# givemeone1astkiss/RNA-MPNN

Measured on AMD Instinct MI355X. Metric: nucleotides/sec (forward), k=30 RNA graphs, higher is better.
Workload: dtype bf16; 1 GPU; C2: batch=256 RNAs, n~U[100,140], k=30, default 10-layer RNAMPNN, P=T; max_len=140, weights=closed-form deterministic init (3,536,900 params), parallelism=dp1

## Files before the change

rna-mpnn_amd/csrc/kernels_mpnn.hip:

```cpp
#include "kernels_bf16.h"
#include "bf16_dev.h"
#include <cstdlib>

static_assert(RN_E_F16 == 1 && RN_P_F16 == 1, "k_resmpnn works on f16 e and f16 P / Q tables");
#if !defined(RN_EXPERIMENTS) && (defined(RM_EXP_NOQ) || defined(RM_EXP_NOESTORE) || defined(RM_EXP_NOELOAD) || defined(RM_EXP_NOMFMA) || defined(RM_EXP_NOGELU) || \
                                 defined(RM_EXP_NOLDS) || defined(RM_EXP_STAGGER) || defined(RM_EXP_PRIO) || defined(RM_WAVES) || defined(RM_RING8) || defined(RM_EDB) || \
                                 defined(RM_QROLL) || defined(RM_NO_EPI_FENCE) || defined(RM_EXP_FWDSWEEP))
#error "experimental variants of k_resmpnn need -DRN_EXPERIMENTS (tools/build_mpnn_variant.sh)"
#endif

#ifndef RM_WAVES
#define RM_WAVES 8
#endif
#if RM_WAVES <= 8 && !defined(RM_QROLL)
#define RM_QFULL 1
#endif
#define RM_LDS_P 131072
#define RM_LDS_BE (RM_LDS_P + RM_WAVES * 1024)
#define RM_LDS_BM (RM_LDS_BE + 512)
#define RM_LDS_GB (RM_LDS_BM + 512)
#define RM_LDS_Z (RM_LDS_GB + 512 + 128)
#define RM_LDS_CTR (RM_LDS_Z + 512)
#define RM_LDS_B0 (RM_LDS_CTR + 16)
#define RM_LDS_BYTES (RM_LDS_B0 + 512)
static_assert(RM_LDS_Z % 256 == 128 && RM_LDS_BYTES <= 160 * 1024, "LDS layout");

__device__ __forceinline__ u32x4* rm_efrag(bf16_t* e, int blk, int lane) { return reinterpret_cast<u32x4*>(e) + (size_t)blk * 512 + lane; }
__device__ __forceinline__ f32x16 rm_ld16(const unsigned char* smem, unsigned off) {
    const f32x4* p = reinterpret_cast<const f32x4*>(smem + off);
    const f32x4 a = p[0], b = p[1], c = p[2], d = p[3];
    return f32x16{a[0], a[1], a[2], a[3], b[0], b[1], b[2], b[3], c[0], c[1], c[2], c[3], d[0], d[1], d[2], d[3]};
}
__device__ __forceinline__ float rm_fma_ll(f16x2 a, f16x2 b, float c) {
    float d;
    asm("v_fma_mix_f32 %0, %1, %2, %3 op_sel_hi:[1,1,0]" : "=v"(d) : "v"(a), "v"(b), "v"(c));
    return d;
}
__device__ __forceinline__ float rm_fma_hh(f16x2 a, f16x2 b, float c) {
    float d;
    asm("v_fma_mix_f32 %0, %1, %2, %3 op_sel:[1,1,0] op_sel_hi:[1,1,0]" : "=v"(d) : "v"(a), "v"(b), "v"(c));
    return d;
}
__device__ __forceinline__ f16x4 rm_h4(unsigned w0, unsigned w1) {
    typedef __attribute__((ext_vector_type(2))) unsigned u32x2_;
    return __builtin_bit_cast(f16x4, u32x2_{w0, w1});
}

#ifdef RM_EXP_NOGELU
#define phi4s(y) (y)
#endif
template <bool DO_EDGE, bool DO_MSG, bool EMBED = false>
__global__ void __launch_bounds__(RM_WAVES * 64, RM_WAVES / 4) k_resmpnn(PackInfo pk, int k, int reverse, const int* __restrict__ nbr, bf16_t* __restrict__ e,
        const bf16_t* __restrict__ p_e, const bf16_t* __restrict__ q_e, const bf16_t* __restrict__ p_m, const bf16_t* __restrict__ q_m,
        const float* __restrict__ h_res, const bf16_t* __restrict__ img_e_g, const float* __restrict__ b2e,
        const bf16_t* __restrict__ img_m_g, const float* __restrict__ b2m, float* __restrict__ agg,
        const float* __restrict__ geomh = nullptr, const float* __restrict__ ee_b0 = nullptr) {
    static_assert(!EMBED || (!DO_EDGE && DO_MSG), "EMBED: the edge embedding (feature.py:386-571) in front of the message of layer 1");
    extern __shared__ __attribute__((aligned(256))) unsigned char smem[];
    u32x4* img_e = reinterpret_cast<u32x4*>(smem);
    u32x4* img_m = img_e + 4096;
    constexpr int NW = RM_WAVES;
    const int tid = threadIdx.x, wave = tid >> 6, lane = tid & 63, r = lane & 31, h = lane >> 5;
    const int ntot = pk.cu[pk.B];
    const int nblocks = ntot;
    const int zero_row = pk.Nmax;
    const bool slot_ok = r < k;
    const int last_idx = ntot * k - 1;

    int blk_end, stride, first, lo = 0;
    if ((gridDim.x & 7) == 0) {
        const int chunk = (nblocks + 7) >> 3, x = blockIdx.x & 7;
        blk_end = min(nblocks, (x + 1) * chunk);
        stride = (gridDim.x >> 3) * NW;
        lo = x * chunk;
        first = lo + (blockIdx.x >> 3) * NW;
    } else {
        blk_end = nblocks; stride = gridDim.x * NW; first = blockIdx.x * NW;
    }
    const int mirror = lo + blk_end - 1;
    auto phys = [&](int b) -> int { return __builtin_amdgcn_readfirstlane(reverse ? mirror - b : b); };
    int* lds_ctr = reinterpret_cast<int*>(smem + RM_LDS_CTR);
    auto claim_issue = [&]() -> int {
        int v = 0;
        if (lane == 0) v = __hip_atomic_fetch_add(lds_ctr, 1, __ATOMIC_RELAXED, __HIP_MEMORY_SCOPE_WORKGROUP);
        return v;
    };
    auto claim_block = [&](int v) -> int {
        const int n = __builtin_amdgcn_readfirstlane(v);
        return first + (n % NW) + (n / NW) * stride;
    };
    int blk = first + wave, nxt = blk + stride;
    u32x4 ef[8];
    unsigned pn_e = 0u, pn_m = 0u;
    int jraw = -1;
    const int b0 = __builtin_amdgcn_readfirstlane(blk < blk_end ? (reverse ? mirror - blk : blk) : 0);
    if (nblocks > 0) {
        const int i0 = b0 * k + r;
        jraw = nbr[i0 > last_idx ? last_idx : i0];
        if (!EMBED) {
#pragma unroll
            for (int s = 0; s < 8; ++s) ef[s] = rm_efrag(e, b0, lane)[64 * s];
        }
        if (DO_EDGE) pn_e = reinterpret_cast<const unsigned*>(p_e + (size_t)b0 * RN_D)[lane];
        if (DO_MSG) pn_m = reinterpret_cast<const unsigned*>(p_m + (size_t)b0 * RN_D)[lane];
    }
    if (DO_EDGE) stage_image_dma<NW * 64>(img_e, reinterpret_cast<const u32x4*>(img_e_g), tid);
    if (EMBED) stage_image_dma<NW * 64, (4 * EMB_KS + 32) * 64>(img_e, reinterpret_cast<const u32x4*>(img_e_g), tid);
    if (DO_MSG) stage_image_dma<NW * 64>(img_m, reinterpret_cast<const u32x4*>(img_m_g), tid);
    if (EMBED && tid >= 256 + 64 && tid < 256 + 64 + 128) reinterpret_cast<float*>(smem + RM_LDS_B0)[tid - 320] = kGA * ee_b0[tid - 320];
    if (tid < 128) {
        reinterpret_cast<float*>(smem + RM_LDS_BE)[tid] = (DO_EDGE || EMBED) ? b2e[tid] : 0.f;
        const float bm = DO_MSG ? b2m[tid] : 0.f;
        const f16x2 bh = cvt_h2(bm, bm);
        reinterpret_cast<unsigned*>(smem + RM_LDS_BM)[tid] = __builtin_bit_cast(unsigned, bh);
        const f16x2 ph = phi2s(bh);
        reinterpret_cast<float*>(smem + RM_LDS_GB)[tid] = (float)bh[0] * (float)ph[0];
    } else if (tid < 256) {
        reinterpret_cast<unsigned*>(smem + RM_LDS_Z)[tid - 128] = 0u;
    } else if (tid == 256) {
        *lds_ctr = 2 * NW;
    }
    dma_landed();
    __syncthreads();
    if (blk >= blk_end) return;

    const unsigned off_pe = RM_LDS_P + wave * 1024 + 64 * h, off_pm = off_pe + 512, off_be = RM_LDS_BE + 64 * h;
    float* lds_pw = reinterpret_cast<float*>(smem + RM_LDS_P + wave * 1024);
    auto stage_p = [&]() {
        if (DO_EDGE) {
            const f16x2 v = __builtin_bit_cast(f16x2, pn_e);
            *reinterpret_cast<f32x2*>(lds_pw + 2 * lane) = f32x2{(float)v[0], (float)v[1]};
        }
        if (DO_MSG) {
            const f16x2 v = __builtin_bit_cast(f16x2, pn_m);
            *reinterpret_cast<f32x2*>(lds_pw + 128 + 2 * lane) = f32x2{(float)v[0], (float)v[1]};
        }
    };
    constexpr int C_FIRST = DO_EDGE ? 0 : 8, C_LAST = DO_MSG ? 15 : 7;
#ifdef RM_EXP_NOLDS
#define RM_FRAG(c, s) (wf[s])
#else
#define RM_FRAG(c, s) (((c) < 8 ? img_e : img_m)[(((c) >> 2) & 1) * 2048 + (((c) & 3) * 8 + (s)) * 64 + lane])
#endif
#define RM_NEXT(c) ((c) == C_LAST ? C_FIRST : (c) + 1)
#define RM_FENCE() __builtin_amdgcn_sched_barrier(0)
#ifdef RM_NO_EPI_FENCE
#define RM_EFENCE() do { } while (0)
#else
#define RM_EFENCE() RM_FENCE()
#endif
#ifdef RM_RING8
#define RM_RING 8
#else
#define RM_RING 4
#endif
    u32x4 q[8], hb[8], wf[8];
    f32x16 T;
    auto gather_q = [&](auto cbc, const bf16_t* table, int jj) {
        constexpr int cb = decltype(cbc)::value;
        const int row = jj >= 0 ? (jj > zero_row ? zero_row : jj) : zero_row;
        const u32x4* src = reinterpret_cast<const u32x4*>(table + (size_t)row * RN_D + 32 * cb + 16 * h);
#ifdef RM_EXP_NOQ
        (void)src; q[2 * cb] = u32x4{0u, 0u, 0u, 0u}; q[2 * cb + 1] = u32x4{0u, 0u, 0u, 0u};
#else
        q[2 * cb] = src[0]; q[2 * cb + 1] = src[1];
#endif
    };
    auto chain = [&](auto cc, auto&& extra) {
        constexpr int c = decltype(cc)::value, kind = c >> 2, cn = RM_NEXT(c);
#pragma unroll
        for (int s = RM_RING; s < 8; ++s) wf[s] = RM_FRAG(c, s);
        RM_FENCE();
        static_for<8>([&](auto sc) {
            constexpr int s = decltype(sc)::value;
#ifdef RM_EXP_NOMFMA
            if constexpr (s == 0) T[0] += __uint_as_float(wf[s][0] ^ (kind == 0 || kind == 2 ? ef[s][0] : hb[s][0]));
            else T[s] += __uint_as_float(wf[s][0] ^ (kind == 0 || kind == 2 ? ef[s][0] : hb[s][0]));
#else
            if constexpr (kind == 3) {
                if constexpr (s == 0) T = mfma32h(hb[0], wf[0], f32x16{0.f, 0.f, 0.f, 0.f, 0.f, 0.f, 0.f, 0.f, 0.f, 0.f, 0.f, 0.f, 0.f, 0.f, 0.f, 0.f});
                else T = mfma32h(hb[s], wf[s], T);
            } else if constexpr (kind == 1) T = mfma32h(wf[s], hb[s], T);
            else T = mfma32h(wf[s], ef[s], T);
#endif
            if constexpr (s < RM_RING) wf[s] = RM_FRAG(cn, s);
            extra(sc);
        });
        asm volatile("" : "+v"(T) :: "memory");
    };
    auto no_extra = [](auto) {};
#ifdef RM_QFULL
#define RM_GQ_ROLL(cb, tab, jj) do { } while (0)
#define RM_GQ_FULL(tab, jj) do { gather_q(std::integral_constant<int, 0>{}, tab, jj); gather_q(std::integral_constant<int, 1>{}, tab, jj); gather_q(std::integral_constant<int, 2>{}, tab, jj); gather_q(std::integral_constant<int, 3>{}, tab, jj); } while (0)
#else
#define RM_GQ_ROLL(cb, tab, jj) gather_q(cb, tab, jj)
#define RM_GQ_FULL(tab, jj) do { } while (0)
#endif
    auto cvt_tile = [&](f16x4 (&x)[4], int next_init) {
#pragma unroll
        for (int v = 0; v < 4; ++v) x[v] = cvt_h4(T[4 * v], T[4 * v + 1], T[4 * v + 2], T[4 * v + 3]);
        asm volatile("" : "+v"(x[0]), "+v"(x[1]), "+v"(x[2]), "+v"(x[3]) :: "memory");
#ifndef RM_EXP_NOLDS
        if (next_init >= 0) T = rm_ld16(smem, (unsigned)next_init);
#endif
    };
    auto epi_first = [&](auto cbc, int next_init) {
        constexpr int cb = decltype(cbc)::value;
        f16x4 x[4];
        cvt_tile(x, next_init);
#pragma unroll
        for (int v = 0; v < 4; ++v) {
            const f16x4 y = x[v] + rm_h4(q[2 * cb + (v >> 1)][2 * (v & 1)], q[2 * cb + (v >> 1)][2 * (v & 1) + 1]);
            const f16x4 g = y * phi4s(y);
            hb[2 * cb + (v >> 1)][2 * (v & 1)] = __builtin_bit_cast(unsigned, lo2(g));
            hb[2 * cb + (v >> 1)][2 * (v & 1) + 1] = __builtin_bit_cast(unsigned, hi2(g));
        }
        RM_EFENCE();
    };
    auto epi_edge = [&](auto obc, int next_init, int gblk) {
        constexpr int ob = decltype(obc)::value;
        f16x4 x[4];
        cvt_tile(x, next_init);
#pragma unroll
        for (int v = 0; v < 4; ++v) {
            const f16x4 ph = phi4s(x[v]);
            const int sp = v >> 1, t = 2 * (v & 1);
            const unsigned o0 = ef[2 * ob + sp][t], o1 = ef[2 * ob + sp][t + 1];
            ef[2 * ob + sp][t] = __builtin_bit_cast(unsigned, __builtin_elementwise_fma(lo2(x[v]), lo2(ph), __builtin_bit_cast(f16x2, o0)));
            ef[2 * ob + sp][t + 1] = __builtin_bit_cast(unsigned, __builtin_elementwise_fma(hi2(x[v]), hi2(ph), __builtin_bit_cast(f16x2, o1)));
#ifndef RM_EXP_NOESTORE
            if (v & 1) rm_efrag(e, gblk, lane)[64 * (2 * ob + sp)] = ef[2 * ob + sp];
#endif
        }
        RM_EFENCE();
    };
    auto epi_mean = [&](auto nbc, int next_init, int gblk, float cabs, float inv, float hres) {
        constexpr int nb = decltype(nbc)::value;
        const unsigned bw = reinterpret_cast<const unsigned*>(smem + RM_LDS_BM)[32 * nb + r];
        const float gbv = reinterpret_cast<const float*>(smem + RM_LDS_GB)[32 * nb + r];
        f16x4 x[4];
        cvt_tile(x, next_init);
        const f16x4 bh = rm_h4(bw, bw);
        float s0 = 0.f, s1 = 0.f;
#pragma unroll
        for (int v = 0; v < 4; ++v) {
            const f16x4 y = x[v] + bh;
            const f16x4 ph = phi4s(y);
            s0 = rm_fma_ll(lo2(y), lo2(ph), s0);
            s1 = rm_fma_hh(lo2(y), lo2(ph), s1);
            s0 = rm_fma_ll(hi2(y), hi2(ph), s0);
            s1 = rm_fma_hh(hi2(y), hi2(ph), s1);
        }
        float sum = s0 + s1;
        sum += __shfl_xor(sum, 32, 64);
        agg[(size_t)gblk * RN_D + 32 * nb + r] = fmaf(sum - cabs * gbv, inv, hres);
        RM_EFENCE();
    };

    f32x4 nrec[7];
    auto load_rec = [&](int jj) {
        const f32x4* src = reinterpret_cast<const f32x4*>(geomh + (size_t)(jj >= 0 ? jj : 0) * RN_GEOMH + 32 * h);
#pragma unroll
        for (int v = 0; v < 7; ++v) nrec[v] = src[v];
    };
    int j = (slot_ok && b0 < ntot) ? jraw : -1;
    if constexpr (EMBED) load_rec(j);
    gather_q(std::integral_constant<int, 0>{}, DO_EDGE ? q_e : q_m, j);
    gather_q(std::integral_constant<int, 1>{}, DO_EDGE ? q_e : q_m, j);
#ifdef RM_QFULL
    gather_q(std::integral_constant<int, 2>{}, DO_EDGE ? q_e : q_m, j);
    gather_q(std::integral_constant<int, 3>{}, DO_EDGE ? q_e : q_m, j);
#endif
    stage_p();
#pragma unroll
    for (int s = 0; s < RM_RING; ++s) wf[s] = RM_FRAG(C_FIRST, s);
    if constexpr (!EMBED) T = rm_ld16(smem, j >= 0 ? (DO_EDGE ? off_pe : off_pm) : (unsigned)RM_LDS_Z);
    RM_FENCE();

#ifdef RM_EXP_STAGGER
    if (wave >= NW / 2) { for (int i = 0; i < RM_EXP_STAGGER; ++i) __builtin_amdgcn_s_sleep(4); }
#endif
#ifdef RM_EXP_PRIO
    if (wave >= NW / 2) __builtin_amdgcn_s_setprio(RM_EXP_PRIO);
#endif
    while (true) {
        const int nblk = nxt;
        const int claim_v = claim_issue();
        const bool has_next = nblk < blk_end;
        const int pblk = phys(blk);
        const int nb_c = phys(has_next ? nblk : blk);
        const int in_ = nb_c * k + r;
        const int jn_raw = nbr[in_ > last_idx ? last_idx : in_];
        if (DO_EDGE) pn_e = reinterpret_cast<const unsigned*>(p_e + (size_t)nb_c * RN_D)[lane];
        if (DO_MSG) pn_m = reinterpret_cast<const unsigned*>(p_m + (size_t)nb_c * RN_D)[lane];
        const bool valid = j >= 0;
        const unsigned vmask = (unsigned)(__ballot(valid) & 0xffffffffull);
        const int cnt = __popc(vmask);
        const float cabs = (float)(32 - cnt);
        const float inv = cnt > 0 ? kGAi * __builtin_amdgcn_rcpf((float)cnt) : 0.f;
        const int a_pe = valid ? (int)off_pe : RM_LDS_Z, a_pm = valid ? (int)off_pm : RM_LDS_Z, a_be = valid ? (int)off_be : RM_LDS_Z;
        const int jn = (slot_ok && nb_c < ntot) ? jn_raw : -1;
        const int a_next = jn >= 0 ? (int)(DO_EDGE ? off_pe : off_pm) : RM_LDS_Z;
#ifdef RM_EDB
        u32x4 efn[8];
#pragma unroll
        for (int s = 0; s < 8; ++s) efn[s] = rm_efrag(e, nb_c, lane)[64 * s];
#endif
        using I0 = std::integral_constant<int, 0>; using I1 = std::integral_constant<int, 1>;
        using I2 = std::integral_constant<int, 2>; using I3 = std::integral_constant<int, 3>;
        RM_FENCE();

        if constexpr (DO_EDGE) {
            chain(std::integral_constant<int, 0>{}, no_extra); RM_GQ_ROLL(I2{}, q_e, j); epi_first(I0{}, a_pe + 128);
            chain(std::integral_constant<int, 1>{}, no_extra); RM_GQ_ROLL(I3{}, q_e, j); epi_first(I1{}, a_pe + 256);
            chain(std::integral_constant<int, 2>{}, no_extra); epi_first(I2{}, a_pe + 384);
            chain(std::integral_constant<int, 3>{}, no_extra); epi_first(I3{}, a_be);
            chain(std::integral_constant<int, 4>{}, no_extra); if constexpr (DO_MSG) RM_GQ_FULL(q_m, j); epi_edge(I0{}, a_be + 128, pblk);
            chain(std::integral_constant<int, 5>{}, no_extra); epi_edge(I1{}, a_be + 256, pblk);
            if constexpr (DO_MSG) {
                chain(std::integral_constant<int, 6>{}, no_extra); RM_GQ_ROLL(I0{}, q_m, j); epi_edge(I2{}, a_be + 384, pblk);
                chain(std::integral_constant<int, 7>{}, no_extra); RM_GQ_ROLL(I1{}, q_m, j); epi_edge(I3{}, a_pm, pblk);
            } else {
                chain(std::integral_constant<int, 6>{}, no_extra); epi_edge(I2{}, a_be + 384, pblk);
                chain(std::integral_constant<int, 7>{}, no_extra);
                stage_p();
                epi_edge(I3{}, a_next, pblk);
                RM_GQ_ROLL(I0{}, q_e, jn); RM_GQ_ROLL(I1{}, q_e, jn); RM_GQ_FULL(q_e, jn);
#pragma unroll
                for (int s = 0; s < 8; ++s) ef[s] = rm_efrag(e, nb_c, lane)[64 * s];
            }
        }
        if constexpr (EMBED) {
            const float* __restrict__ gc = geomh + (size_t)pblk * RN_GEOMH;
            auto catom = [&](int a, int d) { return a < 4 ? gc[3 * a + d] : gc[32 + 3 * (a - 4) + d]; };
            auto cbond = [&](int a, int d) { return a < 3 ? gc[12 + 3 * a + d] : gc[32 + 12 + 3 * (a - 3) + d]; };
            auto cnorm = [&](int a, int d) { return a < 2 ? gc[21 + 3 * a + d] : gc[32 + 21 + 3 * (a - 2) + d]; };
            float nl[28];
#pragma unroll
            for (int v = 0; v < 7; ++v) { nl[4 * v] = nrec[v][0]; nl[4 * v + 1] = nrec[v][1]; nl[4 * v + 2] = nrec[v][2]; nl[4 * v + 3] = nrec[v][3]; }
            float ft[EMB_SLOTS];
#pragma unroll
            for (int a = 0; a < 7; ++a) {
                const float ax = catom(a, 0), ay = catom(a, 1), az = catom(a, 2);
#pragma unroll
                for (int bl = 0; bl < 4; ++bl) {
                    const float dx = nl[3 * bl] - ax, dy = nl[3 * bl + 1] - ay, dz = nl[3 * bl + 2] - az;
                    ft[4 * a + bl] = __builtin_amdgcn_sqrtf(fmaf(dz, dz, fmaf(dy, dy, fmaf(dx, dx, kSEPS))));
                }
            }
#pragma unroll
            for (int a = 0; a < 5; ++a) {
                const float ax = cbond(a, 0), ay = cbond(a, 1), az = cbond(a, 2);
#pragma unroll
                for (int bl = 0; bl < 3; ++bl) ft[28 + 3 * a + bl] = fmaf(az, nl[12 + 3 * bl + 2], fmaf(ay, nl[12 + 3 * bl + 1], ax * nl[12 + 3 * bl]));
            }
#pragma unroll
            for (int a = 0; a < 4; ++a) {
                const float ax = cnorm(a, 0), ay = cnorm(a, 1), az = cnorm(a, 2);
#pragma unroll
                for (int bl = 0; bl < 2; ++bl) ft[43 + 2 * a + bl] = fmaf(az, nl[21 + 3 * bl + 2], fmaf(ay, nl[21 + 3 * bl + 1], ax * nl[21 + 3 * bl]));
            }
#pragma unroll
            for (int pz = 51; pz < EMB_SLOTS; ++pz) ft[pz] = 0.f;
            u32x4 xf[EMB_KS];
#pragma unroll
            for (int s7 = 0; s7 < EMB_KS; ++s7)
#pragma unroll
                for (int t = 0; t < 4; ++t) xf[s7][t] = p_pack2(ft[8 * s7 + 2 * t], ft[8 * s7 + 2 * t + 1]);
            RM_FENCE();
            const unsigned emask = valid ? 0xffffffffu : 0u;
            static_for<4>([&](auto mbc) {
                constexpr int mb = decltype(mbc)::value;
                T = rm_ld16(smem, RM_LDS_B0 + 128 * mb + 64 * h);
#pragma unroll
                for (int s7 = 0; s7 < EMB_KS; ++s7) T = mfma32h(img_e[(mb * EMB_KS + s7) * 64 + lane], xf[s7], T);
                asm volatile("" : "+v"(T) :: "memory");
#pragma unroll
                for (int v = 0; v < 4; ++v) {
                    const f16x4 x = cvt_h4(T[4 * v], T[4 * v + 1], T[4 * v + 2], T[4 * v + 3]);
                    const f16x4 g = x * phi4s(x);
                    hb[2 * mb + (v >> 1)][2 * (v & 1)] = __builtin_bit_cast(unsigned, lo2(g));
                    hb[2 * mb + (v >> 1)][2 * (v & 1) + 1] = __builtin_bit_cast(unsigned, hi2(g));
                }
                RM_FENCE();
            });
            static_for<4>([&](auto obc) {
                constexpr int ob = decltype(obc)::value;
                T = rm_ld16(smem, RM_LDS_BE + 128 * ob + 64 * h);
#pragma unroll
                for (int ks = 0; ks < 8; ++ks) T = mfma32h(img_e[(4 * EMB_KS + ob * 8 + ks) * 64 + lane], hb[ks], T);
                asm volatile("" : "+v"(T) :: "memory");
#pragma unroll
                for (int v = 0; v < 4; ++v) {
                    const f16x4 x = cvt_h4(T[4 * v], T[4 * v + 1], T[4 * v + 2], T[4 * v + 3]);
                    const f16x4 g = x * phi4s(x);
                    const int sp = v >> 1, t = 2 * (v & 1);
                    ef[2 * ob + sp][t] = __builtin_bit_cast(unsigned, lo2(g)) & emask;
                    ef[2 * ob + sp][t + 1] = __builtin_bit_cast(unsigned, hi2(g)) & emask;
                    if (v & 1) rm_efrag(e, pblk, lane)[64 * (2 * ob + sp)] = ef[2 * ob + sp];
                }
                RM_FENCE();
            });
            T = rm_ld16(smem, (unsigned)a_pm);
            RM_FENCE();
        }
        if constexpr (DO_MSG) {
            chain(std::integral_constant<int, 8>{}, no_extra); RM_GQ_ROLL(I2{}, q_m, j); epi_first(I0{}, a_pm + 128);
            chain(std::integral_constant<int, 9>{}, no_extra); RM_GQ_ROLL(I3{}, q_m, j); epi_first(I1{}, a_pm + 256);
            chain(std::integral_constant<int, 10>{}, no_extra); epi_first(I2{}, a_pm + 384);
            chain(std::integral_constant<int, 11>{}, [&](auto sc) {
#if !defined(RM_EXP_NOELOAD) && !defined(RM_EDB)
                if constexpr (!EMBED) { constexpr int s = decltype(sc)::value; ef[s] = rm_efrag(e, nb_c, lane)[64 * s]; }
#endif
            });
            epi_first(I3{}, -1);
            stage_p();
            if constexpr (EMBED) load_rec(jn);
            float hres[4] = {0.f, 0.f, 0.f, 0.f};
            if (h_res) {
#pragma unroll
                for (int nb = 0; nb < 4; ++nb) hres[nb] = h_res[(size_t)pblk * RN_D + 32 * nb + r];
            }
            chain(std::integral_constant<int, 12>{}, no_extra); RM_GQ_FULL(DO_EDGE ? q_e : q_m, jn); epi_mean(I0{}, -1, pblk, cabs, inv, hres[0]);
            chain(std::integral_constant<int, 13>{}, no_extra); epi_mean(I1{}, -1, pblk, cabs, inv, hres[1]);
            chain(std::integral_constant<int, 14>{}, no_extra); RM_GQ_ROLL(I0{}, DO_EDGE ? q_e : q_m, jn); epi_mean(I2{}, -1, pblk, cabs, inv, hres[2]);
            chain(std::integral_constant<int, 15>{}, no_extra); RM_GQ_ROLL(I1{}, DO_EDGE ? q_e : q_m, jn); epi_mean(I3{}, EMBED ? -1 : a_next, pblk, cabs, inv, hres[3]);
        }
#ifdef RM_EDB
#pragma unroll
        for (int s = 0; s < 8; ++s) ef[s] = efn[s];
#endif
        if (!has_next) break;
        blk = nblk;
        nxt = claim_block(claim_v);
        j = jn;
    }
#pragma unroll
    for (int s = 0; s < 8; ++s) asm volatile("" :: "v"(ef[s]));
#pragma unroll
    for (int s = 0; s < 4; ++s) { asm volatile("" :: "v"(q[s])); asm volatile("" :: "v"(wf[s])); }
    if (RM_RING == 8) { for (int s = 4; s < 8; ++s) asm volatile("" :: "v"(wf[s])); }
    asm volatile("" :: "v"(T));
    if constexpr (EMBED) {
#pragma unroll
        for (int v = 0; v < 7; ++v) asm volatile("" :: "v"(nrec[v]));
    }
#undef RM_GQ_ROLL
#undef RM_GQ_FULL
#undef RM_EFENCE
#undef RM_FENCE
#undef RM_NEXT
#undef RM_FRAG
}

bool resmpnn_covers(int k, bool edge1, bool msg_out) { return k > 16 && k <= 32 && !edge1 && !msg_out && !ab_switch("RNAMPNN_MPNN_V3"); }

void launch_resmpnn_bf16(const PackInfo& pk, int k, bool do_edge, bool do_msg, const int* nbr, bf16_t* e, const bf16_t* p_e, const bf16_t* q_e,
                         const bf16_t* p_m, const bf16_t* q_m, MpnnWB we, MpnnWB wm, float* agg, const float* h_res, int reverse, hipStream_t s) {
#ifdef RM_EXP_FWDSWEEP
    reverse = 0;
#endif
    const int max_blocks = pk.Nmax;
    int grid = (max_blocks + RM_WAVES - 1) / RM_WAVES;
    if (grid >= 8) grid = (grid + 7) & ~7;
    const int cus = rn_num_cus();
    if (grid > cus) grid = cus;
    if (grid < 1) grid = 1;
#define RM_LAUNCH(E, M)                                                                                        \
    do {                                                                                                       \
        static DevAttr attr;                                                                                   \
        ensure_dyn_lds((const void*)k_resmpnn<E, M>, RM_LDS_BYTES, attr);                                      \
        hipLaunchKernelGGL((k_resmpnn<E, M>), dim3(grid), dim3(RM_WAVES * 64), RM_LDS_BYTES, s, pk, k, reverse ? 1 : 0, nbr, e, p_e, q_e, p_m, \
                           q_m, h_res, we.img, we.b2p, wm.img, wm.b2p, agg, (const float*)nullptr, (const float*)nullptr); \
    } while (0)
    if (do_edge && do_msg) RM_LAUNCH(true, true);
    else if (do_edge) RM_LAUNCH(true, false);
    else RM_LAUNCH(false, true);
#undef RM_LAUNCH
}

void launch_resmpnn_embed_bf16(const PackInfo& pk, int k, const int* nbr, bf16_t* e, const float* geomh, const bf16_t* ee_img, const float* ee_b0,
                               const float* ee_b1p, const bf16_t* p_m, const bf16_t* q_m, MpnnWB wm, float* agg, const float* h_res, int reverse,
                               hipStream_t s) {
#ifdef RM_EXP_FWDSWEEP
    reverse = 0;
#endif
    int grid = (pk.Nmax + RM_WAVES - 1) / RM_WAVES;
    if (grid >= 8) grid = (grid + 7) & ~7;
    const int cus = rn_num_cus();
    if (grid > cus) grid = cus;
    if (grid < 1) grid = 1;
    static DevAttr attr;
    ensure_dyn_lds((const void*)k_resmpnn<false, true, true>, RM_LDS_BYTES, attr);
    hipLaunchKernelGGL((k_resmpnn<false, true, true>), dim3(grid), dim3(RM_WAVES * 64), RM_LDS_BYTES, s, pk, k, reverse ? 1 : 0, nbr, e, (const bf16_t*)nullptr,
                       (const bf16_t*)nullptr, p_m, q_m, h_res, ee_img, ee_b1p, wm.img, wm.b2p, agg, geomh, ee_b0);
}
```

Measured before the change: 14.04 million nucleotides/s.

## Run plain MPNN kernel with 12 waves and use SGPR-base global addressing

Makes the wave count a template parameter so the plain edge/message kernels launch with 12 waves per workgroup while the embed variant stays at 8, and switches the 12-wave path to rolled Q gathers. It also rewrites global loads and stores to use a uniform scalar base plus a precomputed per-lane byte offset in the global address space, so the compiler can use saddr addressing and keep fewer 64-bit VGPR address pairs. The aim is more latency hiding per CU and lower VGPR and VALU address cost. The trade-off is a tighter register budget at 12 waves, with possible spills, and a rolled gather schedule.

Result: faster. 14.32 million nucleotides/s, median of 6 (+2.0%).

```diff
diff --git a/rna-mpnn_amd/csrc/kernels_mpnn.hip b/rna-mpnn_amd/csrc/kernels_mpnn.hip
--- a/rna-mpnn_amd/csrc/kernels_mpnn.hip
+++ b/rna-mpnn_amd/csrc/kernels_mpnn.hip
@@ -9,23 +9,38 @@
 #error "experimental variants of k_resmpnn need -DRN_EXPERIMENTS (tools/build_mpnn_variant.sh)"
 #endif
 
-#ifndef RM_WAVES
-#define RM_WAVES 8
-#endif
-#if RM_WAVES <= 8 && !defined(RM_QROLL)
-#define RM_QFULL 1
+#ifdef RM_WAVES
+#define RM_NW_PLAIN RM_WAVES
+#define RM_NW_EMBED RM_WAVES
+#else
+#define RM_NW_PLAIN 12
+#define RM_NW_EMBED 8
+#endif
+#ifdef RM_QROLL
+#define RM_QFULL(NW) false
+#else
+#define RM_QFULL(NW) ((NW) <= 8)
 #endif
 #define RM_LDS_P 131072
-#define RM_LDS_BE (RM_LDS_P + RM_WAVES * 1024)
-#define RM_LDS_BM (RM_LDS_BE + 512)
-#define RM_LDS_GB (RM_LDS_BM + 512)
-#define RM_LDS_Z (RM_LDS_GB + 512 + 128)
-#define RM_LDS_CTR (RM_LDS_Z + 512)
-#define RM_LDS_B0 (RM_LDS_CTR + 16)
-#define RM_LDS_BYTES (RM_LDS_B0 + 512)
-static_assert(RM_LDS_Z % 256 == 128 && RM_LDS_BYTES <= 160 * 1024, "LDS layout");
-
-__device__ __forceinline__ u32x4* rm_efrag(bf16_t* e, int blk, int lane) { return reinterpret_cast<u32x4*>(e) + (size_t)blk * 512 + lane; }
+#define RM_LDS_BE(NW) (RM_LDS_P + (NW) * 1024)
+#define RM_LDS_BM(NW) (RM_LDS_BE(NW) + 512)
+#define RM_LDS_GB(NW) (RM_LDS_BM(NW) + 512)
+#define RM_LDS_Z(NW) (RM_LDS_GB(NW) + 512 + 128)
+#define RM_LDS_CTR(NW) (RM_LDS_Z(NW) + 512)
+#define RM_LDS_B0(NW) (RM_LDS_CTR(NW) + 16)
+#define RM_LDS_BYTES(NW) (RM_LDS_B0(NW) + 512)
+static_assert(RM_LDS_Z(RM_NW_PLAIN) % 256 == 128 && RM_LDS_BYTES(RM_NW_PLAIN) <= 160 * 1024, "LDS layout");
+static_assert(RM_LDS_Z(RM_NW_EMBED) % 256 == 128 && RM_LDS_BYTES(RM_NW_EMBED) <= 160 * 1024, "LDS layout");
+
+#define RM_GLOBAL __attribute__((address_space(1)))
+template <class T> __device__ __forceinline__ RM_GLOBAL T* rm_at(T* ubase, unsigned lane_bytes) {
+    RM_GLOBAL const char* g = (RM_GLOBAL const char*)ubase;
+    asm("" : "+s"(g));
+    return (RM_GLOBAL T*)(g + lane_bytes);
+}
+__device__ __forceinline__ RM_GLOBAL u32x4* rm_efrag(bf16_t* e, int ublk, unsigned l16, int s) {
+    return rm_at(reinterpret_cast<u32x4*>(e) + (size_t)ublk * 512 + (s >> 2) * 256, l16) + 64 * (s & 3);
+}
 __device__ __forceinline__ f32x16 rm_ld16(const unsigned char* smem, unsigned off) {
     const f32x4* p = reinterpret_cast<const f32x4*>(smem + off);
     const f32x4 a = p[0], b = p[1], c = p[2], d = p[3];
@@ -49,8 +64,8 @@
 #ifdef RM_EXP_NOGELU
 #define phi4s(y) (y)
 #endif
-template <bool DO_EDGE, bool DO_MSG, bool EMBED = false>
-__global__ void __launch_bounds__(RM_WAVES * 64, RM_WAVES / 4) k_resmpnn(PackInfo pk, int k, int reverse, const int* __restrict__ nbr, bf16_t* __restrict__ e,
+template <int NW, bool DO_EDGE, bool DO_MSG, bool EMBED = false>
+__global__ void __launch_bounds__(NW * 64, NW / 4) k_resmpnn(PackInfo pk, int k, int reverse, const int* __restrict__ nbr, bf16_t* __restrict__ e,
         const bf16_t* __restrict__ p_e, const bf16_t* __restrict__ q_e, const bf16_t* __restrict__ p_m, const bf16_t* __restrict__ q_m,
         const float* __restrict__ h_res, const bf16_t* __restrict__ img_e_g, const float* __restrict__ b2e,
         const bf16_t* __restrict__ img_m_g, const float* __restrict__ b2m, float* __restrict__ agg,
@@ -59,8 +74,10 @@
     extern __shared__ __attribute__((aligned(256))) unsigned char smem[];
     u32x4* img_e = reinterpret_cast<u32x4*>(smem);
     u32x4* img_m = img_e + 4096;
-    constexpr int NW = RM_WAVES;
+    constexpr bool QFULL = RM_QFULL(NW);
     const int tid = threadIdx.x, wave = tid >> 6, lane = tid & 63, r = lane & 31, h = lane >> 5;
+    unsigned l16 = 16u * lane, l4 = 4u * lane, r4 = 4u * r;
+#define RM_LANE_OFFSETS() asm volatile("" : "+v"(l16), "+v"(l4), "+v"(r4))
     const int ntot = pk.cu[pk.B];
     const int nblocks = ntot;
     const int zero_row = pk.Nmax;
@@ -79,7 +96,7 @@
     }
     const int mirror = lo + blk_end - 1;
     auto phys = [&](int b) -> int { return __builtin_amdgcn_readfirstlane(reverse ? mirror - b : b); };
-    int* lds_ctr = reinterpret_cast<int*>(smem + RM_LDS_CTR);
+    int* lds_ctr = reinterpret_cast<int*>(smem + RM_LDS_CTR(NW));
     auto claim_issue = [&]() -> int {
         int v = 0;
         if (lane == 0) v = __hip_atomic_fetch_add(lds_ctr, 1, __ATOMIC_RELAXED, __HIP_MEMORY_SCOPE_WORKGROUP);
@@ -96,27 +113,27 @@
     const int b0 = __builtin_amdgcn_readfirstlane(blk < blk_end ? (reverse ? mirror - blk : blk) : 0);
     if (nblocks > 0) {
         const int i0 = b0 * k + r;
-        jraw = nbr[i0 > last_idx ? last_idx : i0];
+        jraw = *rm_at(nbr, 4u * (unsigned)(i0 > last_idx ? last_idx : i0));
         if (!EMBED) {
 #pragma unroll
-            for (int s = 0; s < 8; ++s) ef[s] = rm_efrag(e, b0, lane)[64 * s];
-        }
-        if (DO_EDGE) pn_e = reinterpret_cast<const unsigned*>(p_e + (size_t)b0 * RN_D)[lane];
-        if (DO_MSG) pn_m = reinterpret_cast<const unsigned*>(p_m + (size_t)b0 * RN_D)[lane];
+            for (int s = 0; s < 8; ++s) ef[s] = *rm_efrag(e, b0, l16, s);
+        }
+        if (DO_EDGE) pn_e = *rm_at(reinterpret_cast<const unsigned*>(p_e + (size_t)b0 * RN_D), l4);
+        if (DO_MSG) pn_m = *rm_at(reinterpret_cast<const unsigned*>(p_m + (size_t)b0 * RN_D), l4);
     }
     if (DO_EDGE) stage_image_dma<NW * 64>(img_e, reinterpret_cast<const u32x4*>(img_e_g), tid);
     if (EMBED) stage_image_dma<NW * 64, (4 * EMB_KS + 32) * 64>(img_e, reinterpret_cast<const u32x4*>(img_e_g), tid);
     if (DO_MSG) stage_image_dma<NW * 64>(img_m, reinterpret_cast<const u32x4*>(img_m_g), tid);
-    if (EMBED && tid >= 256 + 64 && tid < 256 + 64 + 128) reinterpret_cast<float*>(smem + RM_LDS_B0)[tid - 320] = kGA * ee_b0[tid - 320];
+    if (EMBED && tid >= 256 + 64 && tid < 256 + 64 + 128) reinterpret_cast<float*>(smem + RM_LDS_B0(NW))[tid - 320] = kGA * ee_b0[tid - 320];
     if (tid < 128) {
-        reinterpret_cast<float*>(smem + RM_LDS_BE)[tid] = (DO_EDGE || EMBED) ? b2e[tid] : 0.f;
+        reinterpret_cast<float*>(smem + RM_LDS_BE(NW))[tid] = (DO_EDGE || EMBED) ? b2e[tid] : 0.f;
         const float bm = DO_MSG ? b2m[tid] : 0.f;
         const f16x2 bh = cvt_h2(bm, bm);
-        reinterpret_cast<unsigned*>(smem + RM_LDS_BM)[tid] = __builtin_bit_cast(unsigned, bh);
+        reinterpret_cast<unsigned*>(smem + RM_LDS_BM(NW))[tid] = __builtin_bit_cast(unsigned, bh);
         const f16x2 ph = phi2s(bh);
-        reinterpret_cast<float*>(smem + RM_LDS_GB)[tid] = (float)bh[0] * (float)ph[0];
+        reinterpret_cast<float*>(smem + RM_LDS_GB(NW))[tid] = (float)bh[0] * (float)ph[0];
     } else if (tid < 256) {
-        reinterpret_cast<unsigned*>(smem + RM_LDS_Z)[tid - 128] = 0u;
+        reinterpret_cast<unsigned*>(smem + RM_LDS_Z(NW))[tid - 128] = 0u;
     } else if (tid == 256) {
         *lds_ctr = 2 * NW;
     }
@@ -124,7 +141,7 @@
     __syncthreads();
     if (blk >= blk_end) return;
 
-    const unsigned off_pe = RM_LDS_P + wave * 1024 + 64 * h, off_pm = off_pe + 512, off_be = RM_LDS_BE + 64 * h;
+    const unsigned off_pe = RM_LDS_P + wave * 1024 + 64 * h, off_pm = off_pe + 512, off_be = RM_LDS_BE(NW) + 64 * h;
     float* lds_pw = reinterpret_cast<float*>(smem + RM_LDS_P + wave * 1024);
     auto stage_p = [&]() {
         if (DO_EDGE) {
@@ -159,7 +176,7 @@
     auto gather_q = [&](auto cbc, const bf16_t* table, int jj) {
         constexpr int cb = decltype(cbc)::value;
         const int row = jj >= 0 ? (jj > zero_row ? zero_row : jj) : zero_row;
-        const u32x4* src = reinterpret_cast<const u32x4*>(table + (size_t)row * RN_D + 32 * cb + 16 * h);
+        const auto* src = rm_at(reinterpret_cast<const u32x4*>(table), (unsigned)row * (2u * RN_D) + 32u * h) + 4 * cb;
 #ifdef RM_EXP_NOQ
         (void)src; q[2 * cb] = u32x4{0u, 0u, 0u, 0u}; q[2 * cb + 1] = u32x4{0u, 0u, 0u, 0u};
 #else
@@ -189,13 +206,8 @@
         asm volatile("" : "+v"(T) :: "memory");
     };
     auto no_extra = [](auto) {};
-#ifdef RM_QFULL
-#define RM_GQ_ROLL(cb, tab, jj) do { } while (0)
-#define RM_GQ_FULL(tab, jj) do { gather_q(std::integral_constant<int, 0>{}, tab, jj); gather_q(std::integral_constant<int, 1>{}, tab, jj); gather_q(std::integral_constant<int, 2>{}, tab, jj); gather_q(std::integral_constant<int, 3>{}, tab, jj); } while (0)
-#else
-#define RM_GQ_ROLL(cb, tab, jj) gather_q(cb, tab, jj)
-#define RM_GQ_FULL(tab, jj) do { } while (0)
-#endif
+#define RM_GQ_ROLL(cb, tab, jj) do { if constexpr (!QFULL) gather_q(cb, tab, jj); } while (0)
+#define RM_GQ_FULL(tab, jj) do { if constexpr (QFULL) { gather_q(std::integral_constant<int, 0>{}, tab, jj); gather_q(std::integral_constant<int, 1>{}, tab, jj); gather_q(std::integral_constant<int, 2>{}, tab, jj); gather_q(std::integral_constant<int, 3>{}, tab, jj); } } while (0)
     auto cvt_tile = [&](f16x4 (&x)[4], int next_init) {
 #pragma unroll
         for (int v = 0; v < 4; ++v) x[v] = cvt_h4(T[4 * v], T[4 * v + 1], T[4 * v + 2], T[4 * v + 3]);
@@ -229,15 +241,15 @@
             ef[2 * ob + sp][t] = __builtin_bit_cast(unsigned, __builtin_elementwise_fma(lo2(x[v]), lo2(ph), __builtin_bit_cast(f16x2, o0)));
             ef[2 * ob + sp][t + 1] = __builtin_bit_cast(unsigned, __builtin_elementwise_fma(hi2(x[v]), hi2(ph), __builtin_bit_cast(f16x2, o1)));
 #ifndef RM_EXP_NOESTORE
-            if (v & 1) rm_efrag(e, gblk, lane)[64 * (2 * ob + sp)] = ef[2 * ob + sp];
+            if (v & 1) *rm_efrag(e, gblk, l16, 2 * ob + sp) = ef[2 * ob + sp];
 #endif
         }
         RM_EFENCE();
     };
     auto epi_mean = [&](auto nbc, int next_init, int gblk, float cabs, float inv, float hres) {
         constexpr int nb = decltype(nbc)::value;
-        const unsigned bw = reinterpret_cast<const unsigned*>(smem + RM_LDS_BM)[32 * nb + r];
-        const float gbv = reinterpret_cast<const float*>(smem + RM_LDS_GB)[32 * nb + r];
+        const unsigned bw = reinterpret_cast<const unsigned*>(smem + RM_LDS_BM(NW))[32 * nb + r];
+        const float gbv = reinterpret_cast<const float*>(smem + RM_LDS_GB(NW))[32 * nb + r];
         f16x4 x[4];
         cvt_tile(x, next_init);
         const f16x4 bh = rm_h4(bw, bw);
@@ -253,13 +265,13 @@
         }
         float sum = s0 + s1;
         sum += __shfl_xor(sum, 32, 64);
-        agg[(size_t)gblk * RN_D + 32 * nb + r] = fmaf(sum - cabs * gbv, inv, hres);
+        rm_at(agg + (size_t)gblk * RN_D, r4)[32 * nb] = fmaf(sum - cabs * gbv, inv, hres);
         RM_EFENCE();
     };
 
     f32x4 nrec[7];
     auto load_rec = [&](int jj) {
-        const f32x4* src = reinterpret_cast<const f32x4*>(geomh + (size_t)(jj >= 0 ? jj : 0) * RN_GEOMH + 32 * h);
+        const auto* src = rm_at(reinterpret_cast<const f32x4*>(geomh), (unsigned)(jj >= 0 ? jj : 0) * (4u * RN_GEOMH) + 128u * h);
 #pragma unroll
         for (int v = 0; v < 7; ++v) nrec[v] = src[v];
     };
@@ -267,14 +279,14 @@
     if constexpr (EMBED) load_rec(j);
     gather_q(std::integral_constant<int, 0>{}, DO_EDGE ? q_e : q_m, j);
     gather_q(std::integral_constant<int, 1>{}, DO_EDGE ? q_e : q_m, j);
-#ifdef RM_QFULL
-    gather_q(std::integral_constant<int, 2>{}, DO_EDGE ? q_e : q_m, j);
-    gather_q(std::integral_constant<int, 3>{}, DO_EDGE ? q_e : q_m, j);
-#endif
+    if constexpr (QFULL) {
+        gather_q(std::integral_constant<int, 2>{}, DO_EDGE ? q_e : q_m, j);
+        gather_q(std::integral_constant<int, 3>{}, DO_EDGE ? q_e : q_m, j);
+    }
     stage_p();
 #pragma unroll
     for (int s = 0; s < RM_RING; ++s) wf[s] = RM_FRAG(C_FIRST, s);
-    if constexpr (!EMBED) T = rm_ld16(smem, j >= 0 ? (DO_EDGE ? off_pe : off_pm) : (unsigned)RM_LDS_Z);
+    if constexpr (!EMBED) T = rm_ld16(smem, j >= 0 ? (DO_EDGE ? off_pe : off_pm) : (unsigned)RM_LDS_Z(NW));
     RM_FENCE();
 
 #ifdef RM_EXP_STAGGER
@@ -286,25 +298,26 @@
     while (true) {
         const int nblk = nxt;
         const int claim_v = claim_issue();
+        RM_LANE_OFFSETS();
         const bool has_next = nblk < blk_end;
         const int pblk = phys(blk);
         const int nb_c = phys(has_next ? nblk : blk);
         const int in_ = nb_c * k + r;
-        const int jn_raw = nbr[in_ > last_idx ? last_idx : in_];
-        if (DO_EDGE) pn_e = reinterpret_cast<const unsigned*>(p_e + (size_t)nb_c * RN_D)[lane];
-        if (DO_MSG) pn_m = reinterpret_cast<const unsigned*>(p_m + (size_t)nb_c * RN_D)[lane];
+        const int jn_raw = *rm_at(nbr, 4u * (unsigned)(in_ > last_idx ? last_idx : in_));
+        if (DO_EDGE) pn_e = *rm_at(reinterpret_cast<const unsigned*>(p_e + (size_t)nb_c * RN_D), l4);
+        if (DO_MSG) pn_m = *rm_at(reinterpret_cast<const unsigned*>(p_m + (size_t)nb_c * RN_D), l4);
         const bool valid = j >= 0;
         const unsigned vmask = (unsigned)(__ballot(valid) & 0xffffffffull);
         const int cnt = __popc(vmask);
         const float cabs = (float)(32 - cnt);
         const float inv = cnt > 0 ? kGAi * __builtin_amdgcn_rcpf((float)cnt) : 0.f;
-        const int a_pe = valid ? (int)off_pe : RM_LDS_Z, a_pm = valid ? (int)off_pm : RM_LDS_Z, a_be = valid ? (int)off_be : RM_LDS_Z;
+        const int a_pe = valid ? (int)off_pe : RM_LDS_Z(NW), a_pm = valid ? (int)off_pm : RM_LDS_Z(NW), a_be = valid ? (int)off_be : RM_LDS_Z(NW);
         const int jn = (slot_ok && nb_c < ntot) ? jn_raw : -1;
-        const int a_next = jn >= 0 ? (int)(DO_EDGE ? off_pe : off_pm) : RM_LDS_Z;
+        const int a_next = jn >= 0 ? (int)(DO_EDGE ? off_pe : off_pm) : RM_LDS_Z(NW);
 #ifdef RM_EDB
         u32x4 efn[8];
 #pragma unroll
-        for (int s = 0; s < 8; ++s) efn[s] = rm_efrag(e, nb_c, lane)[64 * s];
+        for (int s = 0; s < 8; ++s) efn[s] = *rm_efrag(e, nb_c, l16, s);
 #endif
         using I0 = std::integral_constant<int, 0>; using I1 = std::integral_constant<int, 1>;
         using I2 = std::integral_constant<int, 2>; using I3 = std::integral_constant<int, 3>;
@@ -327,7 +340,7 @@
                 epi_edge(I3{}, a_next, pblk);
                 RM_GQ_ROLL(I0{}, q_e, jn); RM_GQ_ROLL(I1{}, q_e, jn); RM_GQ_FULL(q_e, jn);
 #pragma unroll
-                for (int s = 0; s < 8; ++s) ef[s] = rm_efrag(e, nb_c, lane)[64 * s];
+                for (int s = 0; s < 8; ++s) ef[s] = *rm_efrag(e, nb_c, l16, s);
             }
         }
         if constexpr (EMBED) {
@@ -371,7 +384,7 @@
             const unsigned emask = valid ? 0xffffffffu : 0u;
             static_for<4>([&](auto mbc) {
                 constexpr int mb = decltype(mbc)::value;
-                T = rm_ld16(smem, RM_LDS_B0 + 128 * mb + 64 * h);
+                T = rm_ld16(smem, RM_LDS_B0(NW) + 128 * mb + 64 * h);
 #pragma unroll
                 for (int s7 = 0; s7 < EMB_KS; ++s7) T = mfma32h(img_e[(mb * EMB_KS + s7) * 64 + lane], xf[s7], T);
                 asm volatile("" : "+v"(T) :: "memory");
@@ -386,7 +399,7 @@
             });
             static_for<4>([&](auto obc) {
                 constexpr int ob = decltype(obc)::value;
-                T = rm_ld16(smem, RM_LDS_BE + 128 * ob + 64 * h);
+                T = rm_ld16(smem, RM_LDS_BE(NW) + 128 * ob + 64 * h);
 #pragma unroll
                 for (int ks = 0; ks < 8; ++ks) T = mfma32h(img_e[(4 * EMB_KS + ob * 8 + ks) * 64 + lane], hb[ks], T);
                 asm volatile("" : "+v"(T) :: "memory");
@@ -397,7 +410,7 @@
                     const int sp = v >> 1, t = 2 * (v & 1);
                     ef[2 * ob + sp][t] = __builtin_bit_cast(unsigned, lo2(g)) & emask;
                     ef[2 * ob + sp][t + 1] = __builtin_bit_cast(unsigned, hi2(g)) & emask;
-                    if (v & 1) rm_efrag(e, pblk, lane)[64 * (2 * ob + sp)] = ef[2 * ob + sp];
+                    if (v & 1) *rm_efrag(e, pblk, l16, 2 * ob + sp) = ef[2 * ob + sp];
                 }
                 RM_FENCE();
             });
@@ -410,7 +423,7 @@
             chain(std::integral_constant<int, 10>{}, no_extra); epi_first(I2{}, a_pm + 384);
             chain(std::integral_constant<int, 11>{}, [&](auto sc) {
 #if !defined(RM_EXP_NOELOAD) && !defined(RM_EDB)
-                if constexpr (!EMBED) { constexpr int s = decltype(sc)::value; ef[s] = rm_efrag(e, nb_c, lane)[64 * s]; }
+                if constexpr (!EMBED) { constexpr int s = decltype(sc)::value; ef[s] = *rm_efrag(e, nb_c, l16, s); }
 #endif
             });
             epi_first(I3{}, -1);
@@ -419,8 +432,9 @@
             float hres[4] = {0.f, 0.f, 0.f, 0.f};
             if (h_res) {
 #pragma unroll
-                for (int nb = 0; nb < 4; ++nb) hres[nb] = h_res[(size_t)pblk * RN_D + 32 * nb + r];
+                for (int nb = 0; nb < 4; ++nb) hres[nb] = rm_at(h_res + (size_t)pblk * RN_D, r4)[32 * nb];
             }
+            asm volatile("" : "+v"(r4));
             chain(std::integral_constant<int, 12>{}, no_extra); RM_GQ_FULL(DO_EDGE ? q_e : q_m, jn); epi_mean(I0{}, -1, pblk, cabs, inv, hres[0]);
             chain(std::integral_constant<int, 13>{}, no_extra); epi_mean(I1{}, -1, pblk, cabs, inv, hres[1]);
             chain(std::integral_constant<int, 14>{}, no_extra); RM_GQ_ROLL(I0{}, DO_EDGE ? q_e : q_m, jn); epi_mean(I2{}, -1, pblk, cabs, inv, hres[2]);
@@ -445,6 +459,7 @@
 #pragma unroll
         for (int v = 0; v < 7; ++v) asm volatile("" :: "v"(nrec[v]));
     }
+#undef RM_LANE_OFFSETS
 #undef RM_GQ_ROLL
 #undef RM_GQ_FULL
 #undef RM_EFENCE
@@ -461,7 +476,8 @@
     reverse = 0;
 #endif
     const int max_blocks = pk.Nmax;
-    int grid = (max_blocks + RM_WAVES - 1) / RM_WAVES;
+    constexpr int NW = RM_NW_PLAIN;
+    int grid = (max_blocks + NW - 1) / NW;
     if (grid >= 8) grid = (grid + 7) & ~7;
     const int cus = rn_num_cus();
     if (grid > cus) grid = cus;
@@ -469,8 +485,8 @@
 #define RM_LAUNCH(E, M)                                                                                        \
     do {                                                                                                       \
         static DevAttr attr;                                                                                   \
-        ensure_dyn_lds((const void*)k_resmpnn<E, M>, RM_LDS_BYTES, attr);                                      \
-        hipLaunchKernelGGL((k_resmpnn<E, M>), dim3(grid), dim3(RM_WAVES * 64), RM_LDS_BYTES, s, pk, k, reverse ? 1 : 0, nbr, e, p_e, q_e, p_m, \
+        ensure_dyn_lds((const void*)k_resmpnn<NW, E, M>, RM_LDS_BYTES(NW), attr);                              \
+        hipLaunchKernelGGL((k_resmpnn<NW, E, M>), dim3(grid), dim3(NW * 64), RM_LDS_BYTES(NW), s, pk, k, reverse ? 1 : 0, nbr, e, p_e, q_e, p_m, \
                            q_m, h_res, we.img, we.b2p, wm.img, wm.b2p, agg, (const float*)nullptr, (const float*)nullptr); \
     } while (0)
     if (do_edge && do_msg) RM_LAUNCH(true, true);
@@ -485,13 +501,14 @@
 #ifdef RM_EXP_FWDSWEEP
     reverse = 0;
 #endif
-    int grid = (pk.Nmax + RM_WAVES - 1) / RM_WAVES;
+    constexpr int NW = RM_NW_EMBED;
+    int grid = (pk.Nmax + NW - 1) / NW;
     if (grid >= 8) grid = (grid + 7) & ~7;
     const int cus = rn_num_cus();
     if (grid > cus) grid = cus;
     if (grid < 1) grid = 1;
     static DevAttr attr;
-    ensure_dyn_lds((const void*)k_resmpnn<false, true, true>, RM_LDS_BYTES, attr);
-    hipLaunchKernelGGL((k_resmpnn<false, true, true>), dim3(grid), dim3(RM_WAVES * 64), RM_LDS_BYTES, s, pk, k, reverse ? 1 : 0, nbr, e, (const bf16_t*)nullptr,
+    ensure_dyn_lds((const void*)k_resmpnn<NW, false, true, true>, RM_LDS_BYTES(NW), attr);
+    hipLaunchKernelGGL((k_resmpnn<NW, false, true, true>), dim3(grid), dim3(NW * 64), RM_LDS_BYTES(NW), s, pk, k, reverse ? 1 : 0, nbr, e, (const bf16_t*)nullptr,
                        (const bf16_t*)nullptr, p_m, q_m, h_res, ee_img, ee_b1p, wm.img, wm.b2p, agg, geomh, ee_b0);
 }
```
